# luisdavid64/MRI-Implicit-Neural-Representations

Hardware: AMD Instinct MI355X
Metric: coord-samples/sec (fwd+bwd) fitting 640x368x15-coil k-space; PSNR@1k steps (higher is better)
Workload: dtype f32; 1 GPU; SIREN 5x256 gauss-512 k-space fit, synthetic 640x368x15-coil, L2, Adam; batch_per_gpu=25000, global_batch=25000, parallelism=single, launch=eager

## Files before the change

### include/inr_abi.h

```cpp
#ifndef INR_ABI_H
#define INR_ABI_H

#include <stddef.h>
#include <stdint.h>

#ifdef __cplusplus
extern "C" {
#endif

#define INR_ABI_VERSION 7

#define INR_OK 0
#define INR_ERR_INVALID (-1)
#define INR_ERR_UNSUPPORTED (-2)
#define INR_ERR_HIP (-3)

enum inr_kind {
  INR_KIND_SIREN = 0,
  INR_KIND_FFN = 1,
  INR_KIND_WIRE = 2,
  INR_KIND_FOURIER = 3,
  INR_KIND_MSFOURIER = 4,
  INR_KIND_MSBOUNDED = 5,
  INR_KIND_GABOR = 6,
// ... 85 lines not shown

int inr_plan_create(const inr_net_desc* desc, inr_plan** out);
int inr_plan_destroy(inr_plan* plan);
int inr_plan_sizes(const inr_plan* plan, inr_sizes* out);
int inr_plan_launch_dims(const inr_plan* plan, int64_t B, int64_t* n_tiles, int64_t* n_blocks);
int inr_plan_workspace(const inr_plan* plan, int64_t B, int64_t* step_save_slots, int64_t* n_slabs);
typedef struct inr_step_info {
  int32_t row_split, ncb, grid, rounds, hi, lo, n_hi;
  int32_t hidden_blocks;
} inr_step_info;
int inr_plan_step_info(const inr_plan* plan, int64_t B, inr_step_info* out);
int inr_plan_grad_scale_state(const inr_plan* plan, float* host_out, void* stream);

int inr_pack_params(const inr_plan* plan, const float* params, float* packed, void* stream);

int inr_encode_gauss(const float* coords, const float* enc_B, int64_t B, int32_t E, float* out,
                     void* stream);

int inr_encode_logf(const float* coords, const float* bands, int64_t B, int32_t n_bands, float* out,
                    void* stream);

int inr_forward(const inr_plan* plan, const float* params, const float* packed, const float* x,
                const float* enc_B, int64_t B, float* out, const inr_workspace* ws, void* stream);

int inr_backward(const inr_plan* plan, const float* params, const float* packed, const float* x,
                 const float* enc_B, int64_t B, const float* dout, const inr_workspace* ws,
                 float* grads, void* stream);

int inr_loss_grad(const inr_loss_desc* loss, const float* out, const float* gt, const float* kcoords,
                  const uint8_t* mask, int64_t B, float* loss_out, float* dout, void* stream);
// ... 111 lines not shown
```

### mri-implicit-neural-representations_amd/csrc/inr_api.hip

```cpp
#include <cstring>
#include <mutex>
#include <string>

#include "inr_host.h"

#ifdef INR_STAMPS
namespace inr {
long long* g_stamp_buf = nullptr;
long long g_stamp_cap = 0;
}
using inr::g_stamp_buf;
using inr::g_stamp_cap;
#endif

extern "C" {

static int launch_rs(const inr_plan* plan, const LossDesc& ld, inr::MlpArgs a, int64_t nt, const RsSchedule& sc,
                     hipStream_t st) {
  a.n_tiles = (int)nt;
  a.rs_hi = sc.hi, a.rs_lo = sc.lo, a.rs_x = sc.x, a.rs_rounds = sc.rounds;
  a.tile0 = 0, a.accumulate = 0;
  return hip_done(inr::rs_kernel(sc.ncb)(plan->nd, ld, a, sc.grid, st), "inr row-split kernel launch");
}

// ... 33 lines not shown
    return fail(INR_ERR_INVALID, "%s: stash of %lld floats, the call needs %lld (%lld slots of %d; see "
                "inr_plan_workspace)", who, (long long)(ws->save == nullptr ? 0 : ws->save_floats),
                (long long)need_save, (long long)save_slots, plan->nd.save_floats_per_tile);
  if (n_slabs > 0 && (ws->slabs == nullptr || ws->slab_floats < need_slabs))
    return fail(INR_ERR_INVALID, "%s: %lld slab floats, the call needs %lld (%lld slabs of %d; see "
                "inr_plan_workspace)", who, (long long)(ws->slabs == nullptr ? 0 : ws->slab_floats),
                (long long)need_slabs, (long long)n_slabs, plan->nd.slab_floats);
  return INR_OK;
}

static int launch(const inr_plan* plan, const LossDesc& ld, const inr::MlpArgs& a, int mode, int grid,
                  hipStream_t st) {
  return hip_done(inr::net_kernel(plan->nd)(plan->nd, ld, a, mode, grid, st), "inr mlp kernel launch");
}

static int check_net_call(const char* who, bool null_arg, const inr_plan* plan, bool multi, const float* enc_B,
                          bool need_dist, const float* dist) {
  if (null_arg) return fail(INR_ERR_INVALID, "%s: null argument", who);
  if (!multi && plan->nd.mfn_n > 0) return fail(INR_ERR_INVALID, "%s: multiplicative-filter plans use %s_multi", who, who);
  if (plan->nd.input == IN_GAUSS && enc_B == nullptr) return fail(INR_ERR_INVALID, "%s: enc_B is null", who);
  if (need_dist && plan->nd.bounded && dist == nullptr) return fail(INR_ERR_INVALID, "%s: bounded model needs dist", who);
  if (multi && plan->nd.mfn_n == 0) return fail(INR_ERR_INVALID, "%s: not a multiplicative-filter plan", who);
  return INR_OK;
}

static int check_step_loss(const char* who, const inr_plan* plan, const inr_loss_desc* loss) {
  if (loss->kind < INR_LOSS_L2_HALF || loss->kind > INR_LOSS_CENTER)
    return fail(INR_ERR_INVALID, "%s: loss kind %d", who, loss->kind);
  if (loss->kind >= INR_LOSS_LOGSPACE && plan->nd.out_f != 2)
    return fail(INR_ERR_INVALID, "%s: complex-row losses need out_features == 2", who);
// ... 29 lines not shown
  return INR_OK;
}

int inr_forward(const inr_plan* plan, const float* params, const float* packed, const float* x,
                const float* enc_B, int64_t B, float* out, const inr_workspace* ws, void* stream) {
  const char* who = "inr_forward";
  const bool null_arg = plan == nullptr || params == nullptr || packed == nullptr || x == nullptr || out == nullptr;
  if (int rc = check_net_call(who, null_arg, plan, false, enc_B, false, nullptr)) return rc;
  const bool saving = ws != nullptr && ws->save != nullptr;
  if (plan->nd.hact == ACT_GABOR2D && !saving)
    return fail(INR_ERR_INVALID, "inr_forward: WIRE2D plans need a save buffer (n_tiles * save_floats_per_tile floats)");
  CallLayout c;
  if (int rc = begin_call(plan, B, who, &c)) return rc;
  if (saving)
    if (int rc = check_ws(plan, ws, c.nt, 0, who)) return rc;
  inr::MlpArgs a = net_args(params, packed, x, enc_B, B, c, ws);
  a.out = out;
  a.save_by_block = 0;
  LossDesc ld;
  memset(&ld, 0, sizeof(ld));
  return launch(plan, ld, a, 0, (int)c.nb, (hipStream_t)stream);
}

struct AdamFuse {
  float *params, *m1, *m2, *packed;
  inr::AdamArgs aa;
};

static hipError_t reduce_stage(const inr_plan* plan, const float* slabs, int nb, float* grads, float* loss_out,
                               const float* params, const float* packed, hipStream_t st, const inr::SlabSplit& split,
// ... 31 lines not shown
  hipError_t e = reduce_stage(plan, a.slabs, (int)nb, grads, loss_out, params, packed, st, split, af);
  if (e != hipSuccess) return hip_fail(e, (std::string(who) + ": slab reduction").c_str());
  return INR_OK;
}

int inr_backward(const inr_plan* plan, const float* params, const float* packed, const float* x,
                 const float* enc_B, int64_t B, const float* dout, const inr_workspace* ws,
                 float* grads, void* stream) {
  const char* who = "inr_backward";
  const bool null_arg = plan == nullptr || params == nullptr || packed == nullptr || x == nullptr || dout == nullptr ||
                        ws == nullptr || grads == nullptr;
  if (int rc = check_net_call(who, null_arg, plan, false, enc_B, false, nullptr)) return rc;
  CallLayout c;
  if (int rc = begin_call(plan, B, who, &c)) return rc;
  if (int rc = check_ws(plan, ws, c.nt, c.n_slabs, who)) return rc;
  inr::MlpArgs a = net_args(params, packed, x, enc_B, B, c, ws);
  a.dout = dout;
  a.slabs = ws->slabs;
  a.save_by_block = 0;
  a.dw_gemm = plan->dw_route;
  LossDesc ld;
  memset(&ld, 0, sizeof(ld));
  if (a.dw_gemm == 2) {
    a.dz_state = dz_state_alloc(plan);
    if (a.dz_state == nullptr) return fail(INR_ERR_HIP, "inr_backward: no gradient-scale state on this device");
    if (dz_needs_calibration(plan, 1, B, 0)) {
      int rc = launch(plan, ld, a, 1, (int)c.nb, (hipStream_t)stream);
      if (rc != INR_OK) return rc;
      hipError_t e = inr::launch_dz_roll(a.dz_state + 4, nullptr, (hipStream_t)stream);
      if (e != hipSuccess) return hip_fail(e, "inr_backward: gradient-scale calibration");
// ... 55 lines not shown
  if (e != hipSuccess) return hip_fail(e, (std::string(who) + ": split step").c_str());
  return INR_OK;
}

static int train_step_impl(const inr_plan* plan, const inr_loss_desc* loss, const float* params, const float* packed,
                           const float* x, const float* enc_B, const float* gt, const uint8_t* mask, int64_t B,
                           const inr_workspace* ws, float* grads, float* loss_out, void* stream, const AdamFuse* af) {
  const char* who = "inr_train_step";
  const bool null_arg = plan == nullptr || loss == nullptr || params == nullptr || packed == nullptr || x == nullptr ||
                        gt == nullptr || ws == nullptr || loss_out == nullptr;
  if (int rc = check_net_call(who, null_arg, plan, false, enc_B, false, nullptr)) return rc;
  if (int rc = check_step_loss(who, plan, loss)) return rc;
  CallLayout c;
  if (int rc = begin_call(plan, B, who, &c)) return rc;
  if (int rc = check_ws(plan, ws, c.save_slots, c.n_slabs, who)) return rc;
  inr::MlpArgs a = net_args(params, packed, x, enc_B, B, c, ws);
  a.gt = gt;
  a.mask = mask;
  if (int rc = step_args(plan, ws, who, &a)) return rc;
  LossDesc ld;
  to_loss_desc(loss, &ld);
  return run_fused_step(plan, ld, a, c, grads, loss_out, params, packed, (hipStream_t)stream, who, af);
}

int inr_train_step(const inr_plan* plan, const inr_loss_desc* loss, const float* params, const float* packed,
                   const float* x, const float* enc_B, const float* gt, const uint8_t* mask, int64_t B,
                   const inr_workspace* ws, float* grads, float* loss_out, void* stream) {
  return train_step_impl(plan, loss, params, packed, x, enc_B, gt, mask, B, ws, grads, loss_out, stream, nullptr);
}

int inr_forward_multi(const inr_plan* plan, const float* params, const float* packed, const float* coords,
                      const float* enc_B, const float* dist, int64_t B, float* out, const inr_workspace* ws,
                      int32_t by_block, void* stream) {
  const char* who = "inr_forward_multi";
  const bool null_arg = plan == nullptr || params == nullptr || packed == nullptr || coords == nullptr || out == nullptr ||
                        ws == nullptr;
  if (int rc = check_net_call(who, null_arg, plan, true, enc_B, true, dist)) return rc;
// ... 86 lines not shown
```

### mri-implicit-neural-representations_amd/csrc/inr_api_aux.hip

```cpp
#include <cmath>
#include <cstring>

#include "inr_host.h"

void to_loss_desc(const inr_loss_desc* l, LossDesc* o) {
  memset(o, 0, sizeof(*o));
  o->scale = l->scale == 0.f ? 1.f : l->scale;
  o->cons_w = l->cons_w;
  o->cons_chan = l->cons_chan == 1 ? 1 : 2;
  for (int i = 0; i < INR_MAX_HEADS; ++i) {
    o->cons_lo[i] = l->cons_lo[i];
    o->cons_hi[i] = l->cons_hi[i];
    o->cons_inv[i] = l->cons_inv[i];
  }
  o->kind = l->kind;
  o->eps = l->eps;
  o->sigma = l->sigma;
  o->factor = l->factor;
  o->inv_count = l->inv_count;
  o->hdr_A = l->hdr_A;
}

static bool has_complex_tensors(const NetDesc& nd) {
  for (int l = 0; l < nd.ND; ++l)
// ... 29 lines not shown
  aa.l1 = (float)l1;
  aa.l2 = (float)l2;
  return aa;
}

extern "C" {

int inr_pack_params(const inr_plan* plan, const float* params, float* packed, void* stream) {
  if (plan == nullptr || params == nullptr || packed == nullptr)
    return fail(INR_ERR_INVALID, "inr_pack_params: null argument");
  inr::AdamArgs aa;
  memset(&aa, 0, sizeof(aa));
  aa.do_update = 0;
  hipError_t e = inr::launch_adam_pack(plan->nd, const_cast<float*>(params), nullptr, nullptr, nullptr, packed, aa,
                                       (hipStream_t)stream);
  return hip_done(e, "inr_pack_params");
}

int inr_encode_logf(const float* coords, const float* bands, int64_t B, int32_t n_bands, float* out, void* stream) {
  if (coords == nullptr || bands == nullptr || out == nullptr) return fail(INR_ERR_INVALID, "inr_encode_logf: null argument");
  if (B <= 0 || n_bands <= 0) return fail(INR_ERR_INVALID, "inr_encode_logf: B %lld, n_bands %d", (long long)B, n_bands);
  hipError_t e = inr::launch_encode_logf(coords, bands, B, n_bands, out, (hipStream_t)stream);
  return hip_done(e, "inr_encode_logf");
}

int inr_encode_gauss(const float* coords, const float* enc_B, int64_t B, int32_t E, float* out, void* stream) {
  if (coords == nullptr || enc_B == nullptr || out == nullptr)
    return fail(INR_ERR_INVALID, "inr_encode_gauss: null argument");
  if (B <= 0 || E <= 0) return fail(INR_ERR_INVALID, "inr_encode_gauss: B = %lld, E = %d", (long long)B, E);
  hipError_t e = inr::launch_encode_gauss(coords, enc_B, B, E, out, (hipStream_t)stream);
// ... 455 lines not shown

int inr_adam_step_dev(const inr_plan* plan, float* params, const float* grads, float* exp_avg, float* exp_avg_sq,
                      float* packed, const float* sched, int32_t n_sched, int32_t* step_dev, double beta1,
                      double beta2, double eps, double weight_decay, double l1, double l2, void* stream) {
  if (plan == nullptr || params == nullptr || grads == nullptr || exp_avg == nullptr || exp_avg_sq == nullptr ||
      packed == nullptr || sched == nullptr || step_dev == nullptr)
    return fail(INR_ERR_INVALID, "inr_adam_step_dev: null argument");
  if (n_sched < 1) return fail(INR_ERR_INVALID, "inr_adam_step_dev: empty schedule");
  if (int rc = check_real_penalty(plan, l1, l2, "inr_adam_step_dev")) return rc;
  inr::AdamArgs aa = adam_args(beta1, beta2, eps, weight_decay, l1, l2);
  aa.sched = sched;
  aa.step_dev = step_dev;
  aa.n_sched = n_sched;
  hipError_t e = inr::launch_adam_pack(plan->nd, params, grads, exp_avg, exp_avg_sq, packed, aa, (hipStream_t)stream);
  if (e == hipSuccess) e = inr::launch_step_advance(step_dev, (hipStream_t)stream);
  return hip_done(e, "inr_adam_step_dev");
}

int inr_adam_step(const inr_plan* plan, float* params, const float* grads, float* exp_avg, float* exp_avg_sq,
                  float* packed, double lr, double beta1, double beta2, double eps, double weight_decay,
                  double l1, double l2, int32_t step, void* stream) {
  if (plan == nullptr || params == nullptr || grads == nullptr || exp_avg == nullptr || exp_avg_sq == nullptr ||
      packed == nullptr)
    return fail(INR_ERR_INVALID, "inr_adam_step: null argument");
  if (step < 1) return fail(INR_ERR_INVALID, "inr_adam_step: step %d (counts from 1)", step);
  if (int rc = check_real_penalty(plan, l1, l2, "inr_adam_step")) return rc;
  inr::AdamArgs aa = adam_args(beta1, beta2, eps, weight_decay, l1, l2);
  adam_bias_terms(lr, beta1, beta2, step, &aa.step_size, &aa.bc2_sqrt);
  hipError_t e = inr::launch_adam_pack(plan->nd, params, grads, exp_avg, exp_avg_sq, packed, aa, (hipStream_t)stream);
  return hip_done(e, "inr_adam_step");
}

int inr_reg_grad(const inr_plan* plan, const float* params, float* grads, int64_t lo, int64_t hi, double l1, double l2,
                 const float* l2_dir, void* stream) {
  if (plan == nullptr || params == nullptr || grads == nullptr) return fail(INR_ERR_INVALID, "inr_reg_grad: null argument");
  if (lo < 0 || hi < lo || hi > plan->nd.P)
    return fail(INR_ERR_INVALID, "inr_reg_grad: entries [%lld, %lld) of %d", (long long)lo, (long long)hi, plan->nd.P);
  if (l2 != 0.0 && l2_dir == nullptr && has_complex_tensors(plan->nd))
    return fail(INR_ERR_INVALID, "inr_reg_grad: l2 on a plan with complex64 tensors needs l2_dir (conj(S) / |S|)");
  hipError_t e = inr::launch_reg_grad(plan->nd, params, grads, (int)lo, (int)hi, (float)l1, (float)l2, l2_dir,
                                      (hipStream_t)stream);
  return hip_done(e, "inr_reg_grad");
}

// ... 19 lines not shown
```

### mri-implicit-neural-representations_amd/csrc/inr_aux.h

```cpp
#pragma once
#include "inr_device.h"
#include "inr_mlp_args.h"

namespace inr {

struct AdamArgs {
  int do_update;
  int all_real;
  int has_dead;
  int n_dead;
  int dead_lo[8], dead_hi[8];
  float step_size;
  float bc2_sqrt;
  float omb1;
  float beta2, omb2;
  float eps, weight_decay, l1, l2;
  const float* sched;
  const int* step_dev;
  int n_sched;
};

struct SlabSplit {
  int lo, hi, n2;
  unsigned mask;
// ... 144 lines not shown
```

### mri-implicit-neural-representations_amd/csrc/inr_host.h

```cpp
#pragma once
#include <hip/hip_runtime.h>

#include <cstdint>
#include <mutex>

#include "../../include/inr_abi.h"
#include "inr_aux.h"
#include "inr_dw_gemm.h"
#include "inr_dw_gemm_bf16.h"

#pragma GCC visibility push(hidden)

#ifdef INR_STAMPS
namespace inr {
extern long long* g_stamp_buf;
extern long long g_stamp_cap;
}
#endif

int fail(int code, const char* fmt, ...);
int hip_fail(hipError_t e, const char* what);
inline int hip_done(hipError_t e, const char* what) { return e != hipSuccess ? hip_fail(e, what) : INR_OK; }

inline int round_up(int x, int m) { return (x + m - 1) / m * m; }
// ... 4 lines not shown
  inr_net_desc desc;
  NetDesc nd;
  int64_t packed_floats;
  int dw_route = 0;
  inr::DwGemmArgs gemm;
  inr::SlabSplit gemm_cover;
  mutable std::mutex side_mu;
  mutable hipStream_t side = nullptr;
  mutable int side_dev = -1;
  mutable hipEvent_t fork = nullptr, join = nullptr;
  mutable float* dz_state = nullptr;
  mutable int dz_dev = -1;
  mutable bool dz_ready[2] = {false, false};
  mutable int64_t dz_rows[2] = {0, 0};
  mutable int dz_loss[2] = {-1, -1};
  bool gemm_one_class = false;
  double gemm_enc_cost = 0.0;
};

float* dz_state_alloc(const inr_plan* p);
bool dz_needs_calibration(const inr_plan* p, int kind, int64_t rows, int loss_kind);
void dz_mark(const inr_plan* p, int kind, int64_t rows, int loss_kind);

struct StepSchedule {
  bool split;
  int64_t full, rem, tA;
  inr::DwGemmArgs gA, gB;
  inr::SlabSplit red;
};

// ... 4 lines not shown
struct CallLayout {
  int64_t nt, nb;
  int64_t save_slots, n_slabs;
  bool rs;
  RsSchedule rsched;
  inr::DwGemmArgs plain;
  inr::SlabSplit plain_red;
  StepSchedule step;
  inr::DwGemmBf16Args bf16;
  inr::SlabSplit bf16_red;
};

void call_layout(const inr_plan* plan, int64_t B, CallLayout* c);
int begin_call(const inr_plan* plan, int64_t B, const char* who, CallLayout* c);

void to_loss_desc(const inr_loss_desc* l, LossDesc* o);
int check_real_penalty(const inr_plan* plan, double l1, double l2, const char* who);
void adam_bias_terms(double lr, double beta1, double beta2, int32_t step, float* step_size, float* bc2_sqrt);
inr::AdamArgs adam_args(double beta1, double beta2, double eps, double weight_decay, double l1, double l2);

#pragma GCC visibility pop
```

### mri-implicit-neural-representations_amd/csrc/inr_layout.hip

```cpp
#include <algorithm>
#include <cstdlib>
#include <cstring>

#include "inr_host.h"
#include "inr_w2.h"

static void chunk_tiles(int64_t n, int target, int* tiles_per_chunk, int* n_chunks) {
  target = std::max(1, target);
  *tiles_per_chunk = (int)((n + target - 1) / target);
  *n_chunks = (int)((n + *tiles_per_chunk - 1) / *tiles_per_chunk);
}

static void dw_gemm_chunk(inr::DwGemmArgs& g, int64_t tile0, int64_t tile1, int max_wgs) {
  const int64_t n = tile1 - tile0;
  g.tile0 = (int)tile0, g.n_tiles = (int)tile1;
  g.WBM = 0;
  chunk_tiles(n, max_wgs / std::max(1, inr::dw_gemm_units(g)), &g.tiles_per_chunk, &g.n_chunks);
  if (g.TL == 128 && g.WB == 4 && n > 1 && (int64_t)g.tiles_per_chunk * g.TL < 1024) {
    g.WBM = 2;
    chunk_tiles(n, max_wgs / std::max(1, inr::dw_gemm_units(g)), &g.tiles_per_chunk, &g.n_chunks);
  }
}

constexpr double kEncCost = 1.5;
// ... 116 lines not shown
    c->plain = plan->gemm;
    dw_gemm_chunk(c->plain, 0, nt, 256);
    c->plain_red = plan->gemm_cover;
    c->plain_red.n2 = c->plain.n_chunks;
    step_schedule(plan, nt, c->nb, !(e_overlap != nullptr && e_overlap[0] == '0'), c->plain_red, &c->step);
    int64_t grid = c->nb;
    if (nd.rs) {
      c->rsched = rs_schedule(nt);
      c->rs = rs_enabled(e_rs, nt);
      grid = std::max<int64_t>(grid, c->rsched.grid);
    }
    c->n_slabs = grid + std::max(c->plain.n_chunks, c->step.red.n2);
  }
}

int begin_call(const inr_plan* plan, int64_t B, const char* who, CallLayout* c) {
  if (B <= 0) return fail(INR_ERR_INVALID, "%s: B = %lld", who, (long long)B);
  call_layout(plan, B, c);
  return INR_OK;
}

extern "C" {

int inr_plan_workspace(const inr_plan* plan, int64_t B, int64_t* step_save_slots, int64_t* n_slabs) {
  if (plan == nullptr || step_save_slots == nullptr || n_slabs == nullptr)
    return fail(INR_ERR_INVALID, "inr_plan_workspace: null argument");
  CallLayout c;
  if (int rc = begin_call(plan, B, "inr_plan_launch_dims", &c)) return rc;
  *step_save_slots = c.save_slots, *n_slabs = c.n_slabs;
  return INR_OK;
// ... 3 lines not shown
  if (plan == nullptr || out == nullptr) return fail(INR_ERR_INVALID, "inr_plan_step_info: null argument");
  CallLayout c;
  if (int rc = begin_call(plan, B, "inr_plan_launch_dims", &c)) return rc;
  memset(out, 0, sizeof(*out));
  out->hidden_blocks = plan->nd.NB;
  if (c.rs) {
    const RsSchedule& s = c.rsched;
    out->row_split = 1, out->ncb = s.ncb, out->grid = s.grid, out->rounds = s.rounds;
    out->hi = s.hi, out->lo = s.lo, out->n_hi = s.x;
  } else {
    out->grid = (int32_t)c.nb, out->rounds = (int32_t)((c.nt + c.nb - 1) / c.nb);
  }
  return INR_OK;
}

int inr_plan_launch_dims(const inr_plan* plan, int64_t B, int64_t* n_tiles, int64_t* n_blocks) {
  if (plan == nullptr || n_tiles == nullptr || n_blocks == nullptr)
    return fail(INR_ERR_INVALID, "inr_plan_launch_dims: null argument");
  CallLayout c;
  if (int rc = begin_call(plan, B, "inr_plan_launch_dims", &c)) return rc;
  *n_tiles = c.nt, *n_blocks = c.nb;
  return INR_OK;
}

}
```

### mri-implicit-neural-representations_amd/csrc/inr_params.hip

```cpp
#include <algorithm>
#include <cstdlib>
#include "inr_device.h"
#include "inr_aux.h"
#include "inr_w2.h"
#include "inr_reduce.h"

namespace inr {

struct VirtualPos {
  int n;
  int row[2], col[2];
  float sign[2];
  int bias_row;
};

__device__ __forceinline__ bool locate(const NetDesc& nd, int i, int& l, VirtualPos& vp) {
  vp.n = 0;
  vp.bias_row = -1;
  for (l = 0; l < nd.ND; ++l) {
    const LayerDesc& L = nd.L[l];
    const int off = i - L.w_off;
    if (off >= 0 && off < L.wn) {
      if (L.ltype == LT_REAL || L.ltype == LT_GABOR_MU) {
        vp.n = 1; vp.row[0] = off / L.K; vp.col[0] = off - vp.row[0] * L.K; vp.sign[0] = 1.f;
// ... 169 lines not shown
}

static bool layers_real(const NetDesc& nd, bool with_mu) {
  for (int l = 0; l < nd.ND; ++l)
    if (nd.L[l].ltype != LT_REAL && !(with_mu && nd.L[l].ltype == LT_GABOR_MU)) return false;
  return true;
}

static bool slabs_flat(const NetDesc& nd, const SlabSplit& split) {
  for (int l = 0; l < nd.ND; ++l)
    if (nd.L[l].gw_off != nd.L[l].w_off) return false;
  return layers_real(nd, false) && split.mask == 0 && ((split.lo | split.hi) & 3) == 0 &&
         (split.n3 == 0 || ((split.lo3 | split.hi3) & 3) == 0);
}

hipError_t launch_reduce_slabs(const NetDesc& nd, const float* slabs, int n_blocks, float* grads, float* loss_out,
                               const float* params, const float* packed, hipStream_t st, SlabSplit split) {
  const bool flat = slabs_flat(nd, split);
  if (split.n3 > 0 && !flat) return hipErrorInvalidValue;
  const int grid = (nd.P + 255) / 256;
  if (flat)
    hipLaunchKernelGGL(reduce_slabs_real_kernel, dim3(grid + 1), dim3(256), 0, st, slabs, n_blocks, nd.slab_floats, nd.P,
                       nd.slab_loss_off, grads, loss_out, split);
  else
    hipLaunchKernelGGL(reduce_slabs_kernel, dim3(grid + 1), dim3(256), 0, st, nd, slabs, n_blocks, grads, loss_out, split);
  if (nd.gabor)
    hipLaunchKernelGGL(gabor_finish_kernel, dim3(nd.L[nd.mu0].M, nd.mfn_n + 1), dim3(64), 0, st, nd, slabs, n_blocks,
                       params, packed, grads);
  return hipGetLastError();
}
// ... 45 lines not shown
  } else {
    w2_kperm_inv(k, t, h, j);
    if (l == D - 1)
      img[w2_index(w2_p_last(D, E), t, h * 32 + row, j)] = (__bf16)v;
    else
      img[w2_index(w2_p_fwd(l, E) + (row >> 5), t, h * 32 + (row & 31), j)] = (__bf16)(v * w2_krev(nd, l));
    w2_kperm_inv(row, t, h, j);
    const float vt = v * nd.L[l - 1].omega;
    if (l == D - 1)
      img[w2_index(w2_p_lastT(D, E), k >> 5, h * 32 + (k & 31), j)] = (__bf16)vt;
    else
      img[w2_index(w2_p_T(l, D, E) + (k >> 5), t, h * 32 + (k & 31), j)] = (__bf16)vt;
  }
}

__device__ __forceinline__ float adam_update_entry(const NetDesc& nd, int i, float g, float* __restrict__ params,
                                                   float* __restrict__ m1, float* __restrict__ m2, const AdamArgs& aa) {
  float p = params[i];
  bool live = true;
  if (aa.has_dead) {
    if (aa.n_dead >= 0) {
      for (int r = 0; r < aa.n_dead; ++r)
        if (i >= aa.dead_lo[r] && i < aa.dead_hi[r]) live = false;
    } else {
      for (int l = 0; l < nd.ND; ++l) {
        const LayerDesc& L = nd.L[l];
        if ((i >= L.w_off && i < L.w_off + L.wn) || (i >= L.b_off && i < L.b_off + L.bn)) live = L.live != 0;
      }
    }
  }
  if (aa.do_update && live) {
    if (aa.weight_decay != 0.f) g = fmaf(aa.weight_decay, p, g);
    if (aa.l1 != 0.f) g += aa.l1 * (p > 0.f ? 1.f : (p < 0.f ? -1.f : 0.f));
    if (aa.l2 != 0.f) g = fmaf(2.f * aa.l2, p, g);
    float step_size = aa.step_size, bc2_sqrt = aa.bc2_sqrt;
    if (aa.sched != nullptr) {
      const int t = min(*aa.step_dev, aa.n_sched - 1);
      step_size = aa.sched[2 * t];
      bc2_sqrt = aa.sched[2 * t + 1];
    }
    float m = m1[i], v = m2[i];
    m = m + (g - m) * aa.omb1;
    v = fmaf(g * g, aa.omb2, v * aa.beta2);
    const float denom = sqrtf(v) / bc2_sqrt + aa.eps;
    p = p - step_size * (m / denom);
    m1[i] = m;
    m2[i] = v;
    params[i] = p;
  }
  return p;
}

__device__ __forceinline__ void adam_pack_entry(const NetDesc& nd, int i, float g, float* __restrict__ params,
                                                float* __restrict__ m1, float* __restrict__ m2,
                                                float* __restrict__ packed, const AdamArgs& aa) {
  const float p = adam_update_entry(nd, i, g, params, m1, m2, aa);
  if (aa.all_real) {
    for (int l = 0; l < nd.ND; ++l) {
      const LayerDesc& L = nd.L[l];
      const int off = i - L.w_off;
      if (off >= 0 && off < L.wn) {
        const int row = off / L.K, k = off - row * L.K;
        if (nd.bf16) {
          put_w2(nd, l, packed, row, k, p);
          return;
        }
        put_fwd(nd, L, l, packed, row, k, p);
        if (L.pb_off >= 0) put_tr(L, packed, row, k, p);
        if (nd.rs) put_rs(nd, L, l, packed, row, k, p);
        return;
      }
      const int ob = i - L.b_off;
      if (ob >= 0 && ob < L.bn) {
        if (nd.bf16)
          packed[nd.w2_bias_off + l * 256 + ob] = p * w2_krev(nd, l);
        else
          packed[L.pbias_off + ob] = p;
        return;
      }
    }
    return;
  }
  int l;
  VirtualPos vp;
  if (!locate(nd, i, l, vp)) return;
  const LayerDesc& L = nd.L[l];
  for (int t = 0; t < vp.n; ++t) {
    put_fwd(nd, L, l, packed, vp.row[t], vp.col[t], vp.sign[t] * p);
    if (L.pb_off >= 0) put_tr(L, packed, vp.row[t], vp.col[t], vp.sign[t] * p);
  }
  if (vp.bias_row >= 0) packed[L.pbias_off + vp.bias_row] = p;
}

__global__ __launch_bounds__(256) void adam_pack_kernel(const NetDesc nd, float* __restrict__ params,
                                                        const float* __restrict__ grads, float* __restrict__ m1,
                                                        float* __restrict__ m2, float* __restrict__ packed,
                                                        AdamArgs aa) {
  const int i = blockIdx.x * 256 + threadIdx.x;
  if (i >= nd.P) return;
  adam_pack_entry(nd, i, aa.do_update ? grads[i] : 0.f, params, m1, m2, packed, aa);
}

__global__ __launch_bounds__(256) void reduce_adam_real_kernel(const NetDesc nd, const float* __restrict__ slabs_all,
                                                               int n_blocks_all, float* __restrict__ grads,
                                                               float* __restrict__ loss_out, SlabSplit split,
                                                               float* __restrict__ params, float* __restrict__ m1,
                                                               float* __restrict__ m2, float* __restrict__ packed,
                                                               AdamArgs aa) {
  __shared__ f32x4 part[4][64];
  const int P = nd.P, w = threadIdx.x >> 6;
  const int i4 = (blockIdx.x * 64 + (threadIdx.x & 63)) * 4;
  const f32x4 t = flat_slab_sum(slabs_all, n_blocks_all, nd.slab_floats, P, split, part);
  if (i4 < P) {
    if (w == 0)
      for (int j = 0; j < 4 && i4 + j < P; ++j) grads[i4 + j] = t[j];
    if (i4 + w < P) adam_pack_entry(nd, i4 + w, t[w], params, m1, m2, packed, aa);
  }
  if (loss_out != nullptr && blockIdx.x == gridDim.x - 1)
    loss_words_sum(slabs_all, n_blocks_all, (size_t)nd.slab_floats, nd.slab_loss_off, loss_out);
}

__global__ __launch_bounds__(256) void adam_shard_kernel(const NetDesc nd, float* __restrict__ params,
                                                         const float* __restrict__ grads_shard, float* __restrict__ m1,
                                                         float* __restrict__ m2, int lo, int hi, AdamArgs aa) {
  const int i = lo + blockIdx.x * 256 + threadIdx.x;
  if (i >= hi) return;
  adam_update_entry(nd, i, grads_shard[i - lo], params, m1, m2, aa);
}

__global__ __launch_bounds__(256) void pack_images_real_kernel(const NetDesc nd, const float* __restrict__ params,
                                                               float* __restrict__ packed) {
// ... 101 lines not shown
      lo[m] = lo[i], hi[m] = hi[i], ++m;
    }
  }
  if (m > 8) {
    aa.n_dead = -1;
    return;
  }
  aa.n_dead = m;
  for (int i = 0; i < m; ++i) aa.dead_lo[i] = lo[i], aa.dead_hi[i] = hi[i];
}

hipError_t launch_adam_pack(const NetDesc& nd, float* params, const float* grads, float* m1, float* m2,
                            float* packed, const AdamArgs& aa_in, hipStream_t st) {
  AdamArgs aa = aa_in;
  aa.all_real = layers_real(nd, true);
  adam_dead_ranges(nd, aa);
  const char* force = getenv("INR_PACK_BY_IMAGE");
  const bool big = force != nullptr ? force[0] == '1' : nd.P >= (1 << 18);
  bool by_image = aa.all_real && !nd.bf16 && !nd.rs && !nd.gabor && big;
  int slots = 0;
  for (int l = 0; l < nd.ND && by_image; ++l) {
    const LayerDesc& L = nd.L[l];
    by_image = L.ltype == LT_REAL && L.pf_off >= 0 && (L.pf_off & 3) == 0 && (L.pb_off < 0 || (L.pb_off & 3) == 0) &&
               (L.pbias_off & 3) == 0;
    slots = std::max(slots, L.Kpad8 * L.Mblk * 8 + (L.pb_off >= 0 ? L.Mpad8 * L.Kblk * 8 : 0) + L.Mblk * 8);
  }
  if (by_image) {
    if (aa.do_update)
      hipLaunchKernelGGL(adam_shard_kernel, dim3((nd.P + 255) / 256), dim3(256), 0, st, nd, params, grads, m1, m2, 0, nd.P,
                         aa);
// ... 7 lines not shown
  return hipGetLastError();
}

hipError_t launch_reg_grad(const NetDesc& nd, const float* params, float* grads, int lo, int hi, float l1, float l2,
                           const float* l2_dir, hipStream_t st) {
  if (hi <= lo || (l1 == 0.f && l2 == 0.f)) return hipSuccess;
  hipLaunchKernelGGL(reg_grad_kernel, dim3((hi - lo + 255) / 256), dim3(256), 0, st, nd, params, grads, lo, hi, l1, l2,
                     l2_dir);
  return hipGetLastError();
}

hipError_t launch_adam_shard(const NetDesc& nd, float* params, const float* grads_shard, float* m1, float* m2, int lo,
                             int hi, const AdamArgs& aa_in, hipStream_t st) {
  if (hi <= lo) return hipSuccess;
  AdamArgs aa = aa_in;
  aa.all_real = 0;
  adam_dead_ranges(nd, aa);
  hipLaunchKernelGGL(adam_shard_kernel, dim3((hi - lo + 255) / 256), dim3(256), 0, st, nd, params, grads_shard, m1, m2, lo,
                     hi, aa);
  return hipGetLastError();
}

hipError_t launch_reduce_slabs_adam(const NetDesc& nd, const float* slabs, int n_blocks, float* grads, float* loss_out,
                                    float* params, float* m1, float* m2, float* packed, const AdamArgs& aa_in,
                                    hipStream_t st, SlabSplit split) {
  if (!(slabs_flat(nd, split) && ((split.lo3 | split.hi3) & 3) == 0 && !nd.gabor)) {
    hipError_t e = launch_reduce_slabs(nd, slabs, n_blocks, grads, loss_out, params, packed, st, split);
    if (e != hipSuccess) return e;
    return launch_adam_pack(nd, params, grads, m1, m2, packed, aa_in, st);
  }
  AdamArgs aa = aa_in;
  aa.all_real = 1;
  adam_dead_ranges(nd, aa);
  const int grid = (nd.P + 255) / 256;
  hipLaunchKernelGGL(reduce_adam_real_kernel, dim3(grid + 1), dim3(256), 0, st, nd, slabs, n_blocks, grads, loss_out, split,
                     params, m1, m2, packed, aa);
  return hipGetLastError();
}

}
```

### mri-implicit-neural-representations_amd/csrc/inr_plan.hip

```cpp
#include <cmath>
#include <cstdarg>
#include <cstdio>
#include <cstdlib>
#include <cstring>
#include <new>

#include "inr_host.h"
#include "inr_w2.h"

namespace {

thread_local char g_err[512] = "";

inline int pick_nb(int need, std::initializer_list<int> built) {
  for (int nb : built)
    if (nb >= need) return nb;
  return -1;
}

}

int fail(int code, const char* fmt, ...) {
  va_list ap;
  va_start(ap, fmt);
// ... 24 lines not shown
    return nullptr;
  }
  p->dz_dev = dev;
  return p->dz_state;
}

bool dz_needs_calibration(const inr_plan* p, int kind, int64_t rows, int loss_kind) {
  return !p->dz_ready[kind] || (kind == 0 ? p->dz_loss[0] != loss_kind
                                          : (rows > 2 * p->dz_rows[1] || 2 * rows < p->dz_rows[1]));
}
void dz_mark(const inr_plan* p, int kind, int64_t rows, int loss_kind) {
  p->dz_ready[kind] = true;
  p->dz_rows[kind] = rows;
  p->dz_loss[kind] = loss_kind;
}
static bool dw_gemm_items(const NetDesc& nd, inr::DwGemmArgs* g, inr::SlabSplit* split) {
  memset(g, 0, sizeof(*g));
  split->lo = split->hi = split->n2 = 0;
  split->mask = 0;
  const bool g2d = nd.hact == ACT_GABOR2D;
  if (nd.bf16) return false;
  if (nd.mfn_n != 0) {
    if (nd.NB != 16) return false;
    const int S = nd.mfn_stages, n = nd.mfn_n, HSZ = 16 * 32 * 64;
    if (2 * S - 1 > INR_DWG_MAX_ITEMS) return false;
    g->TL = 64, g->WB = 4;
    g->save_floats_per_tile = nd.save_floats_per_tile, g->slab_floats = nd.slab_floats;
    int k = 0;
    unsigned mask = 0;
    for (int t = 0; t < 2 * S - 1; ++t) {
// ... 437 lines not shown
```

### mri-implicit-neural-representations_amd/inr_mi355x/_lib.py

```python
from __future__ import annotations

import ctypes as C
import os

_HERE = os.path.dirname(os.path.abspath(__file__))
LIB_PATH = os.environ.get("INR_LIB_PATH") or os.path.join(os.path.dirname(_HERE), "lib", "libinr_mi355x.so")

KIND_SIREN, KIND_FFN, KIND_WIRE, KIND_FOURIER, KIND_MSFOURIER, KIND_MSBOUNDED, KIND_GABOR, KIND_KGABOR, KIND_WIRE2D = range(9)
PRECISION_F32, PRECISION_BF16 = 0, 1
ACT_ID, ACT_SIN, ACT_TANH, ACT_RELU, ACT_SIGMOID = 0, 1, 2, 3, 4
ACT_CTANH = 7
INPUT_X, INPUT_GAUSS = 0, 1
LOSS_L2_HALF, LOSS_L1_HALF, LOSS_TANH, LOSS_LOGSPACE, LOSS_HDR, LOSS_MSLE_HALF, LOSS_CENTER = 0, 1, 2, 3, 4, 5, 6
LOSS_WORDS = 512


class NetDesc(C.Structure):
    _fields_ = [("kind", C.c_int32), ("in_features", C.c_int32), ("width", C.c_int32), ("depth", C.c_int32),
                ("out_features", C.c_int32), ("last_act", C.c_int32), ("input", C.c_int32),
                ("enc_size", C.c_int32), ("w0", C.c_float), ("first_omega_0", C.c_float),
                ("hidden_omega_0", C.c_float), ("scale_0", C.c_float), ("precision", C.c_int32),
                ("reserved", C.c_int32 * 3)]


# ... 27 lines not shown
                ("hi", C.c_int32), ("lo", C.c_int32), ("n_hi", C.c_int32), ("hidden_blocks", C.c_int32)]


_P = C.c_void_p
SYMBOLS = {
    "inr_abi_version": (C.c_int, []),
    "inr_last_error": (C.c_int, [C.c_char_p, C.c_size_t]),
    "inr_plan_create": (C.c_int, [C.POINTER(NetDesc), C.POINTER(_P)]),
    "inr_plan_destroy": (C.c_int, [_P]),
    "inr_plan_sizes": (C.c_int, [_P, C.POINTER(Sizes)]),
    "inr_plan_launch_dims": (C.c_int, [_P, C.c_int64, C.POINTER(C.c_int64), C.POINTER(C.c_int64)]),
    "inr_plan_workspace": (C.c_int, [_P, C.c_int64, C.POINTER(C.c_int64), C.POINTER(C.c_int64)]),
    "inr_plan_step_info": (C.c_int, [_P, C.c_int64, C.POINTER(StepInfo)]),
    "inr_plan_grad_scale_state": (C.c_int, [_P, C.POINTER(C.c_float), _P]),
    "inr_pack_params": (C.c_int, [_P, _P, _P, _P]),
    "inr_encode_gauss": (C.c_int, [_P, _P, C.c_int64, C.c_int32, _P, _P]),
    "inr_encode_logf": (C.c_int, [_P, _P, C.c_int64, C.c_int32, _P, _P]),
    "inr_forward": (C.c_int, [_P, _P, _P, _P, _P, C.c_int64, _P, C.POINTER(Workspace), _P]),
    "inr_backward": (C.c_int, [_P, _P, _P, _P, _P, C.c_int64, _P, C.POINTER(Workspace), _P, _P]),
    "inr_loss_grad": (C.c_int, [C.POINTER(LossDesc), _P, _P, _P, _P, C.c_int64, _P, _P, _P]),
    "inr_loss_grad_multi": (C.c_int, [C.POINTER(LossDesc), _P, _P, _P, _P, C.c_int32, C.c_int64, _P, _P, _P]),
    "inr_loss_tv_grad": (C.c_int, [C.POINTER(LossDesc), _P, _P, _P, C.c_int64, C.c_int64, C.c_int64, C.c_int64, C.c_float,
                                   _P, _P, _P]),
    "inr_tv_grad": (C.c_int, [_P, C.c_int64, C.c_int64, C.c_int64, C.c_int64, C.c_float, _P, _P, _P]),
    "inr_center_pairs_grad": (C.c_int, [_P, _P, _P, _P, C.c_int64, C.c_int64, C.c_float, _P, _P, _P]),
    "inr_train_step": (C.c_int, [_P, C.POINTER(LossDesc), _P, _P, _P, _P, _P, _P, C.c_int64, C.POINTER(Workspace), _P,
                                 _P, _P]),
    "inr_plan_heads": (C.c_int, [_P, C.POINTER(C.c_int32)]),
    "inr_plan_set_bounds": (C.c_int, [_P, C.POINTER(C.c_float), C.POINTER(C.c_float), C.c_int32]),
    "inr_forward_multi": (C.c_int, [_P, _P, _P, _P, _P, _P, C.c_int64, _P, C.POINTER(Workspace), C.c_int32, _P]),
# ... 79 lines not shown
```

Before: 67.78 million coord-samples/s.

## Lazily repack only the weight images the fused step reads

```diff
diff --git a/include/inr_abi.h b/include/inr_abi.h
--- a/include/inr_abi.h
+++ b/include/inr_abi.h
@@ -123,6 +123,19 @@
 
 int inr_pack_params(const inr_plan* plan, const float* params, float* packed, void* stream);
 
+#define INR_IMG_FWD 1
+#define INR_IMG_TR 2
+#define INR_IMG_RS 4
+#define INR_IMG_EV_PACK 0
+#define INR_IMG_EV_UPDATE 1
+#define INR_IMG_EV_READ 2
+#define INR_IMG_CALL_FORWARD 0
+#define INR_IMG_CALL_BACKWARD 1
+#define INR_IMG_CALL_STEP 2
+int inr_plan_image_sets(const inr_plan* plan, int32_t* valid, int32_t* lazy);
+int inr_image_sets_after(int32_t valid, int32_t event, int32_t sets);
+int inr_image_sets_read(int32_t call, int32_t row_split);
+
 int inr_encode_gauss(const float* coords, const float* enc_B, int64_t B, int32_t E, float* out,
                      void* stream);
 
diff --git a/mri-implicit-neural-representations_amd/csrc/inr_api.hip b/mri-implicit-neural-representations_amd/csrc/inr_api.hip
--- a/mri-implicit-neural-representations_amd/csrc/inr_api.hip
+++ b/mri-implicit-neural-representations_amd/csrc/inr_api.hip
@@ -71,6 +71,20 @@
   return hip_done(inr::net_kernel(plan->nd)(plan->nd, ld, a, mode, grid, st), "inr mlp kernel launch");
 }
 
+static int ensure_images(const inr_plan* plan, const float* params, const float* packed, int reads, hipStream_t st,
+                         const char* who) {
+  const int stale = plan->nd.rs ? reads & ~plan->img_valid : 0;
+  if (stale == 0) return INR_OK;
+  inr::AdamArgs aa;
+  memset(&aa, 0, sizeof(aa));
+  aa.skip_sets = inr::IMG_ALL & ~stale;
+  hipError_t e = inr::launch_adam_pack(plan->nd, const_cast<float*>(params), nullptr, nullptr, nullptr,
+                                       const_cast<float*>(packed), aa, st);
+  if (e != hipSuccess) return hip_fail(e, (std::string(who) + ": re-pack of stale weight images").c_str());
+  images_note(plan, IMG_EV_READ, stale, st);
+  return INR_OK;
+}
+
 static int check_net_call(const char* who, bool null_arg, const inr_plan* plan, bool multi, const float* enc_B,
                           bool need_dist, const float* dist) {
   if (null_arg) return fail(INR_ERR_INVALID, "%s: null argument", who);
@@ -130,6 +144,8 @@
   if (int rc = begin_call(plan, B, who, &c)) return rc;
   if (saving)
     if (int rc = check_ws(plan, ws, c.nt, 0, who)) return rc;
+  if (int rc = ensure_images(plan, params, packed, image_sets_read(IMG_CALL_FORWARD, false), (hipStream_t)stream, who))
+    return rc;
   inr::MlpArgs a = net_args(params, packed, x, enc_B, B, c, ws);
   a.out = out;
   a.save_by_block = 0;
@@ -191,6 +207,8 @@
   CallLayout c;
   if (int rc = begin_call(plan, B, who, &c)) return rc;
   if (int rc = check_ws(plan, ws, c.nt, c.n_slabs, who)) return rc;
+  if (int rc = ensure_images(plan, params, packed, image_sets_read(IMG_CALL_BACKWARD, false), (hipStream_t)stream, who))
+    return rc;
   inr::MlpArgs a = net_args(params, packed, x, enc_B, B, c, ws);
   a.dout = dout;
   a.slabs = ws->slabs;
@@ -276,13 +294,21 @@
   CallLayout c;
   if (int rc = begin_call(plan, B, who, &c)) return rc;
   if (int rc = check_ws(plan, ws, c.save_slots, c.n_slabs, who)) return rc;
+  const int reads = image_sets_read(IMG_CALL_STEP, c.rs);
+  if (int rc = ensure_images(plan, params, packed, reads, (hipStream_t)stream, who)) return rc;
   inr::MlpArgs a = net_args(params, packed, x, enc_B, B, c, ws);
   a.gt = gt;
   a.mask = mask;
   if (int rc = step_args(plan, ws, who, &a)) return rc;
   LossDesc ld;
   to_loss_desc(loss, &ld);
-  return run_fused_step(plan, ld, a, c, grads, loss_out, params, packed, (hipStream_t)stream, who, af);
+  if (af == nullptr || grads == nullptr)
+    return run_fused_step(plan, ld, a, c, grads, loss_out, params, packed, (hipStream_t)stream, who, af);
+  AdamFuse lazy = *af;
+  lazy.aa.skip_sets = image_sets_skip(plan, reads, (hipStream_t)stream);
+  int rc = run_fused_step(plan, ld, a, c, grads, loss_out, params, packed, (hipStream_t)stream, who, &lazy);
+  if (rc == INR_OK) images_note(plan, IMG_EV_UPDATE, inr::IMG_ALL & ~lazy.aa.skip_sets, (hipStream_t)stream);
+  return rc;
 }
 
 int inr_train_step(const inr_plan* plan, const inr_loss_desc* loss, const float* params, const float* packed,
diff --git a/mri-implicit-neural-representations_amd/csrc/inr_api_aux.hip b/mri-implicit-neural-representations_amd/csrc/inr_api_aux.hip
--- a/mri-implicit-neural-representations_amd/csrc/inr_api_aux.hip
+++ b/mri-implicit-neural-representations_amd/csrc/inr_api_aux.hip
@@ -67,6 +67,7 @@
   aa.do_update = 0;
   hipError_t e = inr::launch_adam_pack(plan->nd, const_cast<float*>(params), nullptr, nullptr, nullptr, packed, aa,
                                        (hipStream_t)stream);
+  if (e == hipSuccess) images_note(plan, IMG_EV_PACK, inr::IMG_ALL, (hipStream_t)stream);
   return hip_done(e, "inr_pack_params");
 }
 
@@ -552,6 +553,7 @@
   aa.n_sched = n_sched;
   hipError_t e = inr::launch_adam_pack(plan->nd, params, grads, exp_avg, exp_avg_sq, packed, aa, (hipStream_t)stream);
   if (e == hipSuccess) e = inr::launch_step_advance(step_dev, (hipStream_t)stream);
+  if (e == hipSuccess) images_note(plan, IMG_EV_PACK, inr::IMG_ALL, (hipStream_t)stream);
   return hip_done(e, "inr_adam_step_dev");
 }
 
@@ -566,6 +568,7 @@
   inr::AdamArgs aa = adam_args(beta1, beta2, eps, weight_decay, l1, l2);
   adam_bias_terms(lr, beta1, beta2, step, &aa.step_size, &aa.bc2_sqrt);
   hipError_t e = inr::launch_adam_pack(plan->nd, params, grads, exp_avg, exp_avg_sq, packed, aa, (hipStream_t)stream);
+  if (e == hipSuccess) images_note(plan, IMG_EV_PACK, inr::IMG_ALL, (hipStream_t)stream);
   return hip_done(e, "inr_adam_step");
 }
 
diff --git a/mri-implicit-neural-representations_amd/csrc/inr_aux.h b/mri-implicit-neural-representations_amd/csrc/inr_aux.h
--- a/mri-implicit-neural-representations_amd/csrc/inr_aux.h
+++ b/mri-implicit-neural-representations_amd/csrc/inr_aux.h
@@ -4,9 +4,13 @@
 
 namespace inr {
 
+enum { IMG_FWD = 1, IMG_TR = 2, IMG_RS = 4, IMG_ALL = 7 };
+
 struct AdamArgs {
   int do_update;
+  int skip_sets;
   int all_real;
+  int flat_order;
   int has_dead;
   int n_dead;
   int dead_lo[8], dead_hi[8];
diff --git a/mri-implicit-neural-representations_amd/csrc/inr_host.h b/mri-implicit-neural-representations_amd/csrc/inr_host.h
--- a/mri-implicit-neural-representations_amd/csrc/inr_host.h
+++ b/mri-implicit-neural-representations_amd/csrc/inr_host.h
@@ -42,6 +42,8 @@
   mutable bool dz_ready[2] = {false, false};
   mutable int64_t dz_rows[2] = {0, 0};
   mutable int dz_loss[2] = {-1, -1};
+  mutable int img_valid = inr::IMG_ALL;
+  mutable bool img_eager = false;
   bool gemm_one_class = false;
   double gemm_enc_cost = 0.0;
 };
@@ -76,6 +78,15 @@
 void call_layout(const inr_plan* plan, int64_t B, CallLayout* c);
 int begin_call(const inr_plan* plan, int64_t B, const char* who, CallLayout* c);
 
+enum { IMG_EV_PACK = 0, IMG_EV_UPDATE = 1, IMG_EV_READ = 2 };
+enum { IMG_CALL_FORWARD = 0, IMG_CALL_BACKWARD = 1, IMG_CALL_STEP = 2 };
+int image_sets_after(int valid, int event, int sets);
+int image_sets_read(int call, bool row_split);
+bool lazy_pack_enabled();
+bool stream_capturing(hipStream_t st);
+int image_sets_skip(const inr_plan* plan, int reads, hipStream_t st);
+void images_note(const inr_plan* plan, int event, int sets, hipStream_t st);
+
 void to_loss_desc(const inr_loss_desc* l, LossDesc* o);
 int check_real_penalty(const inr_plan* plan, double l1, double l2, const char* who);
 void adam_bias_terms(double lr, double beta1, double beta2, int32_t step, float* step_size, float* bc2_sqrt);
diff --git a/mri-implicit-neural-representations_amd/csrc/inr_layout.hip b/mri-implicit-neural-representations_amd/csrc/inr_layout.hip
--- a/mri-implicit-neural-representations_amd/csrc/inr_layout.hip
+++ b/mri-implicit-neural-representations_amd/csrc/inr_layout.hip
@@ -154,6 +154,23 @@
   }
 }
 
+int image_sets_after(int valid, int event, int sets) {
+  sets &= inr::IMG_ALL;
+  if (event == IMG_EV_UPDATE) return sets;
+  return (valid | sets) & inr::IMG_ALL;
+}
+
+int image_sets_read(int call, bool row_split) {
+  if (call == IMG_CALL_FORWARD) return inr::IMG_FWD;
+  if (call == IMG_CALL_BACKWARD) return inr::IMG_FWD | inr::IMG_TR;
+  return row_split ? inr::IMG_RS : (inr::IMG_FWD | inr::IMG_TR);
+}
+
+bool lazy_pack_enabled() {
+  const char* e = getenv("INR_LAZY_PACK");
+  return e != nullptr && e[0] == '1';
+}
+
 int begin_call(const inr_plan* plan, int64_t B, const char* who, CallLayout* c) {
   if (B <= 0) return fail(INR_ERR_INVALID, "%s: B = %lld", who, (long long)B);
   call_layout(plan, B, c);
@@ -187,6 +204,18 @@
   return INR_OK;
 }
 
+int inr_image_sets_after(int32_t valid, int32_t event, int32_t sets) { return image_sets_after(valid, event, sets); }
+
+int inr_image_sets_read(int32_t call, int32_t row_split) { return image_sets_read(call, row_split != 0); }
+
+int inr_plan_image_sets(const inr_plan* plan, int32_t* valid, int32_t* lazy) {
+  if (plan == nullptr || valid == nullptr || lazy == nullptr)
+    return fail(INR_ERR_INVALID, "inr_plan_image_sets: null argument");
+  *valid = plan->img_valid;
+  *lazy = plan->nd.rs && !plan->img_eager && lazy_pack_enabled() ? 1 : 0;
+  return INR_OK;
+}
+
 int inr_plan_launch_dims(const inr_plan* plan, int64_t B, int64_t* n_tiles, int64_t* n_blocks) {
   if (plan == nullptr || n_tiles == nullptr || n_blocks == nullptr)
     return fail(INR_ERR_INVALID, "inr_plan_launch_dims: null argument");
diff --git a/mri-implicit-neural-representations_amd/csrc/inr_params.hip b/mri-implicit-neural-representations_amd/csrc/inr_params.hip
--- a/mri-implicit-neural-representations_amd/csrc/inr_params.hip
+++ b/mri-implicit-neural-representations_amd/csrc/inr_params.hip
@@ -207,6 +207,15 @@
          (split.n3 == 0 || ((split.lo3 | split.hi3) & 3) == 0);
 }
 
+static bool layers_flat_order(const NetDesc& nd) {
+  int off = 0;
+  for (int l = 0; l < nd.ND; ++l) {
+    if (nd.L[l].w_off != off || nd.L[l].b_off != off + nd.L[l].wn) return false;
+    off += nd.L[l].wn + nd.L[l].bn;
+  }
+  return off == nd.P;
+}
+
 hipError_t launch_reduce_slabs(const NetDesc& nd, const float* slabs, int n_blocks, float* grads, float* loss_out,
                                const float* params, const float* packed, hipStream_t st, SlabSplit split) {
   const bool flat = slabs_flat(nd, split);
@@ -282,9 +291,9 @@
   }
 }
 
-__device__ __forceinline__ float adam_update_entry(const NetDesc& nd, int i, float g, float* __restrict__ params,
-                                                   float* __restrict__ m1, float* __restrict__ m2, const AdamArgs& aa) {
-  float p = params[i];
+__device__ __forceinline__ float adam_update_loaded(const NetDesc& nd, int i, float g, float p, float m, float v,
+                                                    float* __restrict__ params, float* __restrict__ m1,
+                                                    float* __restrict__ m2, const AdamArgs& aa) {
   bool live = true;
   if (aa.has_dead) {
     if (aa.n_dead >= 0) {
@@ -307,7 +316,6 @@
       step_size = aa.sched[2 * t];
       bc2_sqrt = aa.sched[2 * t + 1];
     }
-    float m = m1[i], v = m2[i];
     m = m + (g - m) * aa.omb1;
     v = fmaf(g * g, aa.omb2, v * aa.beta2);
     const float denom = sqrtf(v) / bc2_sqrt + aa.eps;
@@ -319,23 +327,40 @@
   return p;
 }
 
-__device__ __forceinline__ void adam_pack_entry(const NetDesc& nd, int i, float g, float* __restrict__ params,
-                                                float* __restrict__ m1, float* __restrict__ m2,
-                                                float* __restrict__ packed, const AdamArgs& aa) {
-  const float p = adam_update_entry(nd, i, g, params, m1, m2, aa);
+__device__ __forceinline__ float adam_update_entry(const NetDesc& nd, int i, float g, float* __restrict__ params,
+                                                   float* __restrict__ m1, float* __restrict__ m2, const AdamArgs& aa) {
+  const bool upd = aa.do_update != 0;
+  return adam_update_loaded(nd, i, g, params[i], upd ? m1[i] : 0.f, upd ? m2[i] : 0.f, params, m1, m2, aa);
+}
+
+struct LayerWalk {
+  int l0, i_last;
+};
+__device__ __forceinline__ LayerWalk layer_walk(const NetDesc& nd, const AdamArgs& aa, int first) {
+  LayerWalk lw = {0, 0x7fffffff};
+  if (aa.flat_order) {
+    while (lw.l0 < nd.ND - 1 && nd.L[lw.l0].b_off + nd.L[lw.l0].bn <= first) ++lw.l0;
+    lw.i_last = first + 255;
+  }
+  return lw;
+}
+
+__device__ __forceinline__ void pack_entry(const NetDesc& nd, int i, float p, float* __restrict__ packed, const AdamArgs& aa,
+                                           const LayerWalk& lw) {
+  const int skip = aa.skip_sets;
   if (aa.all_real) {
-    for (int l = 0; l < nd.ND; ++l) {
+    for (int l = lw.l0; l < nd.ND; ++l) {
       const LayerDesc& L = nd.L[l];
       const int off = i - L.w_off;
       if (off >= 0 && off < L.wn) {
-        const int row = off / L.K, k = off - row * L.K;
+        const int row = (L.K & (L.K - 1)) == 0 ? off >> (31 - __clz(L.K)) : off / L.K, k = off - row * L.K;
         if (nd.bf16) {
           put_w2(nd, l, packed, row, k, p);
           return;
         }
-        put_fwd(nd, L, l, packed, row, k, p);
-        if (L.pb_off >= 0) put_tr(L, packed, row, k, p);
-        if (nd.rs) put_rs(nd, L, l, packed, row, k, p);
+        if (!(skip & IMG_FWD)) put_fwd(nd, L, l, packed, row, k, p);
+        if (!(skip & IMG_TR) && L.pb_off >= 0) put_tr(L, packed, row, k, p);
+        if (!(skip & IMG_RS) && nd.rs) put_rs(nd, L, l, packed, row, k, p);
         return;
       }
       const int ob = i - L.b_off;
@@ -346,6 +371,7 @@
           packed[L.pbias_off + ob] = p;
         return;
       }
+      if (L.b_off + L.bn > lw.i_last) return;
     }
     return;
   }
@@ -360,13 +386,20 @@
   if (vp.bias_row >= 0) packed[L.pbias_off + vp.bias_row] = p;
 }
 
+__device__ __forceinline__ void adam_pack_entry(const NetDesc& nd, int i, float g, float* __restrict__ params,
+                                                float* __restrict__ m1, float* __restrict__ m2,
+                                                float* __restrict__ packed, const AdamArgs& aa, const LayerWalk& lw) {
+  pack_entry(nd, i, adam_update_entry(nd, i, g, params, m1, m2, aa), packed, aa, lw);
+}
+
 __global__ __launch_bounds__(256) void adam_pack_kernel(const NetDesc nd, float* __restrict__ params,
                                                         const float* __restrict__ grads, float* __restrict__ m1,
                                                         float* __restrict__ m2, float* __restrict__ packed,
                                                         AdamArgs aa) {
   const int i = blockIdx.x * 256 + threadIdx.x;
+  const LayerWalk lw = layer_walk(nd, aa, blockIdx.x * 256);
   if (i >= nd.P) return;
-  adam_pack_entry(nd, i, aa.do_update ? grads[i] : 0.f, params, m1, m2, packed, aa);
+  adam_pack_entry(nd, i, aa.do_update ? grads[i] : 0.f, params, m1, m2, packed, aa, lw);
 }
 
 __global__ __launch_bounds__(256) void reduce_adam_real_kernel(const NetDesc nd, const float* __restrict__ slabs_all,
@@ -376,13 +409,18 @@
                                                                float* __restrict__ m2, float* __restrict__ packed,
                                                                AdamArgs aa) {
   __shared__ f32x4 part[4][64];
-  const int P = nd.P, w = threadIdx.x >> 6;
-  const int i4 = (blockIdx.x * 64 + (threadIdx.x & 63)) * 4;
+  __shared__ f32x4 sum4[64];
+  const int P = nd.P, i = blockIdx.x * 256 + threadIdx.x;
+  float p = 0.f, m = 0.f, v = 0.f;
+  if (i < P) p = params[i], m = m1[i], v = m2[i];
   const f32x4 t = flat_slab_sum(slabs_all, n_blocks_all, nd.slab_floats, P, split, part);
-  if (i4 < P) {
-    if (w == 0)
-      for (int j = 0; j < 4 && i4 + j < P; ++j) grads[i4 + j] = t[j];
-    if (i4 + w < P) adam_pack_entry(nd, i4 + w, t[w], params, m1, m2, packed, aa);
+  if (threadIdx.x < 64) sum4[threadIdx.x] = t;
+  const LayerWalk lw = layer_walk(nd, aa, blockIdx.x * 256);
+  __syncthreads();
+  if (i < P) {
+    const float g = reinterpret_cast<const float*>(sum4)[threadIdx.x];
+    grads[i] = g;
+    pack_entry(nd, i, adam_update_loaded(nd, i, g, p, m, v, params, m1, m2, aa), packed, aa, lw);
   }
   if (loss_out != nullptr && blockIdx.x == gridDim.x - 1)
     loss_words_sum(slabs_all, n_blocks_all, (size_t)nd.slab_floats, nd.slab_loss_off, loss_out);
@@ -514,6 +552,7 @@
                             float* packed, const AdamArgs& aa_in, hipStream_t st) {
   AdamArgs aa = aa_in;
   aa.all_real = layers_real(nd, true);
+  aa.flat_order = aa.all_real && layers_flat_order(nd);
   adam_dead_ranges(nd, aa);
   const char* force = getenv("INR_PACK_BY_IMAGE");
   const bool big = force != nullptr ? force[0] == '1' : nd.P >= (1 << 18);
@@ -551,7 +590,7 @@
                              int hi, const AdamArgs& aa_in, hipStream_t st) {
   if (hi <= lo) return hipSuccess;
   AdamArgs aa = aa_in;
-  aa.all_real = 0;
+  aa.all_real = aa.flat_order = 0;
   adam_dead_ranges(nd, aa);
   hipLaunchKernelGGL(adam_shard_kernel, dim3((hi - lo + 255) / 256), dim3(256), 0, st, nd, params, grads_shard, m1, m2, lo,
                      hi, aa);
@@ -568,6 +607,7 @@
   }
   AdamArgs aa = aa_in;
   aa.all_real = 1;
+  aa.flat_order = layers_flat_order(nd);
   adam_dead_ranges(nd, aa);
   const int grid = (nd.P + 255) / 256;
   hipLaunchKernelGGL(reduce_adam_real_kernel, dim3(grid + 1), dim3(256), 0, st, nd, slabs, n_blocks, grads, loss_out, split,
diff --git a/mri-implicit-neural-representations_amd/csrc/inr_plan.hip b/mri-implicit-neural-representations_amd/csrc/inr_plan.hip
--- a/mri-implicit-neural-representations_amd/csrc/inr_plan.hip
+++ b/mri-implicit-neural-representations_amd/csrc/inr_plan.hip
@@ -62,6 +62,29 @@
   p->dz_rows[kind] = rows;
   p->dz_loss[kind] = loss_kind;
 }
+bool stream_capturing(hipStream_t st) {
+  hipStreamCaptureStatus cs = hipStreamCaptureStatusNone;
+  return hipStreamIsCapturing(st, &cs) == hipSuccess && cs != hipStreamCaptureStatusNone;
+}
+
+int image_sets_skip(const inr_plan* plan, int reads, hipStream_t st) {
+  if (!plan->nd.rs) return 0;
+  if (stream_capturing(st)) {
+    plan->img_eager = true;
+    return 0;
+  }
+  return plan->img_eager || !lazy_pack_enabled() ? 0 : (inr::IMG_ALL & ~reads);
+}
+
+void images_note(const inr_plan* plan, int event, int sets, hipStream_t st) {
+  if (!plan->nd.rs) return;
+  if (stream_capturing(st)) {
+    plan->img_eager = true;
+    return;
+  }
+  plan->img_valid = image_sets_after(plan->img_valid, event, sets);
+}
+
 static bool dw_gemm_items(const NetDesc& nd, inr::DwGemmArgs* g, inr::SlabSplit* split) {
   memset(g, 0, sizeof(*g));
   split->lo = split->hi = split->n2 = 0;
diff --git a/mri-implicit-neural-representations_amd/inr_mi355x/_lib.py b/mri-implicit-neural-representations_amd/inr_mi355x/_lib.py
--- a/mri-implicit-neural-representations_amd/inr_mi355x/_lib.py
+++ b/mri-implicit-neural-representations_amd/inr_mi355x/_lib.py
@@ -8,6 +8,9 @@
 
 KIND_SIREN, KIND_FFN, KIND_WIRE, KIND_FOURIER, KIND_MSFOURIER, KIND_MSBOUNDED, KIND_GABOR, KIND_KGABOR, KIND_WIRE2D = range(9)
 PRECISION_F32, PRECISION_BF16 = 0, 1
+IMG_FWD, IMG_TR, IMG_RS, IMG_ALL = 1, 2, 4, 7
+IMG_EV_PACK, IMG_EV_UPDATE, IMG_EV_READ = 0, 1, 2
+IMG_CALL_FORWARD, IMG_CALL_BACKWARD, IMG_CALL_STEP = 0, 1, 2
 ACT_ID, ACT_SIN, ACT_TANH, ACT_RELU, ACT_SIGMOID = 0, 1, 2, 3, 4
 ACT_CTANH = 7
 INPUT_X, INPUT_GAUSS = 0, 1
@@ -65,6 +68,9 @@
     "inr_plan_step_info": (C.c_int, [_P, C.c_int64, C.POINTER(StepInfo)]),
     "inr_plan_grad_scale_state": (C.c_int, [_P, C.POINTER(C.c_float), _P]),
     "inr_pack_params": (C.c_int, [_P, _P, _P, _P]),
+    "inr_plan_image_sets": (C.c_int, [_P, C.POINTER(C.c_int32), C.POINTER(C.c_int32)]),
+    "inr_image_sets_after": (C.c_int, [C.c_int32, C.c_int32, C.c_int32]),
+    "inr_image_sets_read": (C.c_int, [C.c_int32, C.c_int32]),
     "inr_encode_gauss": (C.c_int, [_P, _P, C.c_int64, C.c_int32, _P, _P]),
     "inr_encode_logf": (C.c_int, [_P, _P, C.c_int64, C.c_int32, _P, _P]),
     "inr_forward": (C.c_int, [_P, _P, _P, _P, _P, C.c_int64, _P, C.POINTER(Workspace), _P]),
```

New measurement: 68.54 million coord-samples/s (median of 6 runs). +1.1%, better.
